# Parcels-code/Parcels

Hardware: AMD Instinct MI355X
Metric: RK4 particle-steps/sec (higher is better)
Workload: dtype f64

## Files before the change

### include/parcels_hip.h

```cpp
#ifndef PARCELS_HIP_H
#define PARCELS_HIP_H

#include <stdint.h>

#ifdef __cplusplus
extern "C" {
#endif

#define PK_ABI_VERSION 9
#define PK_MAX_GRIDS 4
#define PK_MAX_FIELDS 64
#define PK_MAX_KERNELS 8
#define PK_MAX_EXTRA 8
#define PK_NUM_STATE_CODES 80
#define PK_MAX_TWE 1024

typedef struct pk_ctx pk_ctx;

#define PK_F32 0
#define PK_F64 1
#define PK_I8 2
#define PK_U8 3
#define PK_I16 4
#define PK_U16 5
// ... 37 lines not shown
#define PK_KERNEL_USER0 40
#define PK_MAX_USER_KERNELS 8

int32_t pk_abi_version(void);
int32_t pk_init(int32_t device, pk_ctx** out);
int32_t pk_destroy(pk_ctx* ctx);
const char* pk_last_error(const pk_ctx* ctx);

int32_t pk_set_option(pk_ctx* ctx, const char* name, int32_t value);

int32_t pk_upload_stats(pk_ctx* ctx, double* out4);

int32_t pk_unpack_stats(pk_ctx* ctx, double* out4);

int32_t pk_host_stage_selftest(void);

typedef struct pk_device_info {
    char name[128];
    char arch[64];
    int32_t compute_units;
    int32_t wavefront_size;
    int32_t lds_bytes_per_block;
    int32_t clock_khz;
    int64_t total_mem;
    int64_t free_mem;
} pk_device_info;
int32_t pk_get_device_info(pk_ctx* ctx, pk_device_info* out);

typedef struct pk_grid_desc {
    int32_t kind;
// ... 316 lines not shown
```

### parcels_amd/_hip.py

```python

from __future__ import annotations

import ctypes as C
import os
import subprocess

_HERE = os.path.dirname(os.path.abspath(__file__))
LIB_PATH = os.environ.get("PARCELS_HIP_LIB", os.path.join(_HERE, "libparcels_hip.so"))

PK_ABI_VERSION = 9
PK_USER_RIDE, PK_USER_SAMPLES_UV, PK_USER_SAMPLES_UVW, PK_USER_UX, PK_USER_KEY_UX = 1, 2, 4, 8, 12
PK_USER_SIGMA, PK_USER_KEY_SIGMA = 16, 16
PK_F32, PK_F64 = 0, 1
PK_I8, PK_U8, PK_I16, PK_U16, PK_I32 = 2, 3, 4, 5, 6
PK_MAX_GRIDS, PK_MAX_FIELDS, PK_MAX_KERNELS, PK_NUM_STATE_CODES = 4, 64, 8, 80
PK_MAX_EXTRA = 8
PK_MAX_TWE = 1024
PK_KERNEL_SAMPLE_FIELD = 10
PK_KERNEL_ADVECTION_RK2_3D_CROCO = 11
PK_KERNEL_SAMPLE_SIGMA_CROCO = 12
PK_KERNEL_USER0 = 40
PK_EVAL_MASKED = 0x10000
PK_COMM_ID_BYTES = 128
PK_OP_MIN, PK_OP_MAX, PK_OP_SUM = 0, 1, 2
# ... 300 lines not shown
    "pk_interact_host_order",
    "pk_interact_sources",
    "pk_interact_prologue",
    "pk_interact_attract",
    "pk_interact_merge",
    "pk_interact_epilogue",
    "pk_particles_density",
    "pk_particles_cells",
    "pk_particles_connectivity",
    "pk_random_fill",
    "pk_measure_copy_bandwidth",
    "pk_set_option",
    "pk_upload_stats",
    "pk_unpack_stats",
    "pk_host_stage_selftest",
    "pk_particles_snapshot_filtered",
    "pk_comm_unique_id",
    "pk_comm_init",
    "pk_comm_destroy",
    "pk_comm_info",
    "pk_comm_allreduce_i64",
    "pk_comm_allgather_i64",
    "pk_gather_rows_to_root",
    "pk_allgather_output",
    "pk_gathered_fetch",
]

_lib = None


# ... 176 lines not shown
```

### parcels_amd/csrc/pk_api.hip

```cpp
#include "pk_api_ctx.h"

#include <rocprim/rocprim.hpp>

using namespace pkapi;

namespace pkapi {
std::string g_init_error;
}

namespace pk {

PK_DEV unsigned long long order_double(double v) {
    unsigned long long b = (unsigned long long)__double_as_longlong(v);
    return (b & 0x8000000000000000ull) ? ~b : (b | 0x8000000000000000ull);
}

__global__ void __launch_bounds__(64) clock_probe_kernel(unsigned long long* out, unsigned long long ticks) {
    if (threadIdx.x != 0) return;
    const unsigned long long r0 = __builtin_amdgcn_s_memrealtime();
    const unsigned long long c0 = __builtin_readcyclecounter();
    unsigned long long r = r0;
    while (r - r0 < ticks) {
        __builtin_amdgcn_s_sleep(8);
        r = __builtin_amdgcn_s_memrealtime();
// ... 341 lines not shown
        g_init_error = "device index out of range";
        return -2;
    }
    pk_ctx* ctx = new pk_ctx();
    ctx->device = device;
    if (const char* e = getenv("PK_SORT_HORIZONTAL")) ctx->sort_horizontal_major = atoi(e);
    if (const char* e = getenv("PK_NO_SPECIAL")) ctx->no_special = atoi(e);
    if (const char* e = getenv("PK_NO_CELL_CACHE")) ctx->no_cell_cache = atoi(e);
    if (const char* e = getenv("PK_NO_HASH_DIR")) ctx->no_hash_dir = atoi(e);
    if (const char* e = getenv("PK_NO_CELL_TABLE")) ctx->no_cell_table = atoi(e);
    if (const char* e = getenv("PK_NO_FAST")) ctx->no_fast = atoi(e);
    if (const char* e = getenv("PK_NO_FAST_CGRID")) ctx->no_fast_cgrid = atoi(e);
    if (const char* e = getenv("PK_NO_VELOCITY_PAIRS")) ctx->no_velocity_pairs = atoi(e);
    if (const char* e = getenv("PK_VELOCITY_PAIRS")) ctx->no_velocity_pairs = !atoi(e);
    ctx->no_block_cache = getenv("PK_NO_BLOCK_CACHE") != nullptr;
    *out = ctx;
    PK_HIP(ctx, hipSetDevice(device));
    PK_HIP(ctx, hipGetDeviceProperties(&ctx->prop, device));
    PK_HIP(ctx, hipStreamCreateWithFlags(&ctx->compute, hipStreamNonBlocking));
    PK_HIP(ctx, hipStreamCreateWithFlags(&ctx->copy, hipStreamNonBlocking));
    PK_HIP(ctx, hipEventCreate(&ctx->ev0));
    PK_HIP(ctx, hipEventCreate(&ctx->ev1));
    PK_HIP(ctx, hipEventCreate(&ctx->ev2));
    PK_HIP(ctx, hipEventCreate(&ctx->ev_p0));
    PK_HIP(ctx, hipEventCreate(&ctx->ev_p1));
    for (int k = 0; k < PK_STAGE_BUFFERS; k++) PK_HIP(ctx, hipEventCreateWithFlags(&ctx->stage_ev[k], hipEventDisableTiming));
    PK_HIP(ctx, hipMalloc((void**)&ctx->d_counters, sizeof(DCounters)));
    PK_HIP(ctx, hipMalloc((void**)&ctx->d_twe, sizeof(unsigned long long) * PK_MAX_TWE));
    PK_HIP(ctx, hipMalloc((void**)&ctx->d_twe_found, sizeof(unsigned long long) * TWE_FOUND_SLOTS));
    PK_HIP(ctx, hipMalloc((void**)&ctx->d_twe_hit, sizeof(unsigned int) * PK_MAX_TWE));
    PK_HIP(ctx, hipMalloc((void**)&ctx->d_summary, sizeof(unsigned long long) * (PK_NUM_STATE_CODES + 2)));
    PK_HIP(ctx, hipHostMalloc((void**)&ctx->h_counters, sizeof(DCounters), hipHostMallocDefault));
    PK_HIP(ctx, hipHostMalloc((void**)&ctx->h_summary, sizeof(unsigned long long) * (PK_NUM_STATE_CODES + 2), hipHostMallocDefault));
    PK_HIP(ctx, hipMalloc((void**)&ctx->d_clk, sizeof(unsigned long long) * 32));
    PK_HIP(ctx, hipMalloc((void**)&ctx->d_tstats, sizeof(unsigned long long) * 3));
    PK_HIP(ctx, hipHostMalloc((void**)&ctx->h_clk, sizeof(unsigned long long) * 32, hipHostMallocDefault));
    return 0;
}

int32_t pk_set_option(pk_ctx* ctx, const char* name, int32_t value) {
    if (!ctx || !name) return -2;
    const std::string n(name);
    if (n == "fast_path") ctx->no_fast = !value;
    else if (n == "fast_cgrid") ctx->no_fast_cgrid = !value;
    else if (n == "velocity_pairs") ctx->no_velocity_pairs = !value;
    else if (n == "clock_probe") ctx->clock_probe = value;
    else if (n == "special_programs") ctx->no_special = !value;
// ... 7 lines not shown
        ctx->block_cache = value;
    }
    else if (n == "miss_lanes") {
        if (value < -1 || value > 64) return ctx->fail("pk_set_option: miss_lanes is -1 (planned), 0 (never) or the most missing lanes of a wavefront, up to 64");
        ctx->miss_lanes = value;
    }
    else if (n == "fast_grid") {
        if (value < 0) return ctx->fail("pk_set_option: fast_grid is 0 (planned) or the largest number of workgroups of the persistent A-grid launch");
        ctx->fast_grid = value;
    }
    else if (n == "unpack_chunk_values") {
        if (value < 0) return ctx->fail("pk_set_option: unpack_chunk_values is 0 (what fits a staging chunk) or the most values per staged chunk of a packed level");
        ctx->unpack_chunk_values = value == 0 ? 0 : std::max(16, value / 16 * 16);
    }
    else if (n == "unpack_timing") ctx->unpack_timing = value != 0;
    else return ctx->fail("pk_set_option: unknown option '" + n + "'");
    return 0;
}

int32_t pk_upload_stats(pk_ctx* ctx, double* out4) {
    if (!ctx || !out4) return -2;
    out4[0] = ctx->stage_fill_s;
    out4[1] = ctx->stage_wait_s;
    out4[2] = ctx->stage_bytes_total;
    out4[3] = (double)pkhost::copy_threads();
    return 0;
}

static void free_snapshots(pk_ctx* ctx) {
    for (auto& sn : ctx->snap) {
        if (sn.in_flight && sn.done) (void)hipEventSynchronize(sn.done);
// ... 28 lines not shown
    for (hipEvent_t e : ctx->unpack_ev) (void)hipEventDestroy(e);
    for (hipEvent_t e : ctx->unpack_ev_free) (void)hipEventDestroy(e);
    if (ctx->tab_a.d) (void)hipFree(ctx->tab_a.d);
    if (ctx->tab_c.d) (void)hipFree(ctx->tab_c.d);
    if (ctx->d_ct2) (void)hipFree(ctx->d_ct2);
    if (ctx->d_vp) (void)hipFree(ctx->d_vp);
    if (ctx->d_sigma) (void)hipFree(ctx->d_sigma);
    if (ctx->d_counters) (void)hipFree(ctx->d_counters);
    if (ctx->d_twe) (void)hipFree(ctx->d_twe);
    if (ctx->d_twe_found) (void)hipFree(ctx->d_twe_found);
    if (ctx->d_twe_hit) (void)hipFree(ctx->d_twe_hit);
    if (ctx->d_desc) (void)hipFree(ctx->d_desc);
    if (ctx->h_desc) (void)hipHostFree(ctx->h_desc);
    if (ctx->d_summary) (void)hipFree(ctx->d_summary);
    if (ctx->h_counters) (void)hipHostFree(ctx->h_counters);
    if (ctx->h_summary) (void)hipHostFree(ctx->h_summary);
    (void)pk_comm_destroy(ctx);
    neighbors_free(ctx->nbr);
    interact_free(ctx->inter);
    if (ctx->sel.d_flag) (void)hipFree(ctx->sel.d_flag);
    if (ctx->sel.d_offs) (void)hipFree(ctx->sel.d_offs);
    if (ctx->sel.d_tmp) (void)hipFree(ctx->sel.d_tmp);
    if (ctx->d_clk) (void)hipFree(ctx->d_clk);
    if (ctx->d_tstats) (void)hipFree(ctx->d_tstats);
    if (ctx->h_clk) (void)hipHostFree(ctx->h_clk);
    for (int k = 0; k < PK_STAGE_BUFFERS; k++) {
        if (ctx->stage[k]) (void)hipHostFree(ctx->stage[k]);
        if (ctx->stage_ev[k]) (void)hipEventDestroy(ctx->stage_ev[k]);
    }
    if (ctx->ev0) (void)hipEventDestroy(ctx->ev0);
// ... 1304 lines not shown
    const CoordTable& T = ctx->tab_a;
    if (int32_t rc = coord_table(ctx, ctx->tab_a, U.d.grid, prm->fU, U.time.data(), f.has_time_interval ? f.nt : 0,
                                 {{g.d.depth, g.d.has_z ? g.d.nz : 0}, {g.d.lat, g.d.has_y ? g.d.ny : 0}, {g.d.lon, g.d.nx}}, 60 * 1024))
        return rc;
    if (!T.ok) return 0;
    const double inv_deg2m = 1.0 / g.d.deg2m;
    if (!(g.d.deg2m > 1e-100 && g.d.deg2m < 1e100) || !std::isfinite(inv_deg2m)) return 0;
    F.grid = U.d.grid;
    F.has_ti = f.has_time_interval;
    F.has_z = g.d.has_z; F.has_y = g.d.has_y; F.has_x = g.d.has_x;
    F.spherical = g.d.spherical;
    F.nt = f.nt;
    F.nslots = f.nslots;
    F.gnz = g.d.nz; F.gny = g.d.ny; F.gnx = g.d.nx;
    ravel_strides(g.d, F.ex, F.ey, F.ez);
    F.st_z = (uint32_t)f.st_z;
    F.st_y = (uint32_t)f.st_y;
    F.dyb = fy ? (uint32_t)(f.st_y * esz) : 0u;
    F.dzb = fz ? (uint32_t)(f.st_z * esz) : 0u;
    F.lds_time = T.off[0]; F.lds_depth = T.off[1]; F.lds_lat = T.off[2]; F.lds_lon = T.off[3];
    F.lds_n = T.off[4];
    F.lvl_b = (int64_t)lvl_b;
    F.U = (const char*)U.d.data; F.V = (const char*)V.d.data; F.W = W ? (const char*)W->d.data : nullptr;
    F.tab = T.d;
    F.tlen = f.tlen; F.t0 = f.tfirst; F.t1 = f.tlast;
    F.z0 = g.d.zfirst; F.z1 = g.d.zlast; F.y0 = g.d.yfirst; F.y1 = g.d.ylast; F.x0 = g.d.xfirst; F.x1 = g.d.xlast;
    F.deg2m = g.d.deg2m;
    F.inv_deg2m = inv_deg2m;
    F.ok = 1;
    return 0;
// ... 310 lines not shown
        p.lds = (size_t)a.fast.lds_n * 2 * sizeof(double);
        const bool lp_kernel = fast_prog == PROG_RK4 && !ride;
        const size_t lp_lds = (p.lds + (size_t)FAST_LP_BYTES + 2047) / 2048 * 2048;
        const bool lp_fits = 2 * lp_lds <= (size_t)160 * 1024;
        int mode = ctx->block_cache;
        if (ctx->no_block_cache && mode != 2) mode = 0;
        if (mode == 2 && !(lp_kernel && lp_fits))
            return ctx->fail(!lp_kernel ? "block_cache 2: only the library's 2-D A-grid kernel (AdvectionRK4 without user kernels) has the level-pair cache"
                                        : "block_cache 2: the coordinate tables leave no room for the level-pair cache at 16 waves per CU");
        if (mode < 0) mode = lp_kernel && lp_fits ? 2 : 1;
        if (mode == 2) {
            p.lp = FAST_LP_CACHE;
            a.fast.lds_blk = a.fast.lds_n;
            a.fast.miss_lanes = ctx->miss_lanes < 0 ? FAST_MISS_LANES_DEFAULT : ctx->miss_lanes;
            p.lds += (size_t)FAST_LP_BYTES;
        } else if (mode == 0 && lp_kernel && !ctx->no_block_cache) {
            p.lp = FAST_LP_REGS;
            a.fast.lds_blk = 0;
        } else {
            const bool blk = mode == 1 && fast_prog != PROG_RK4_3D && p.lds + (size_t)FAST_BLK_BYTES <= 64 * 1024;
            a.fast.lds_blk = blk ? a.fast.lds_n : 0;
            if (blk) p.lds += (size_t)FAST_BLK_BYTES;
        }
    } else {
        if (int32_t rc = fill_fastc(ctx, prm, a, fast_prog, prm->have_guess0 || us.assume_guessed, p.lds)) return rc;
        if (!a.fastc.ok) return 0;
        p.kernel = fast_prog == PROG_RK4_3D ? DEDICATED_C3 : DEDICATED_C2;
    }
    p.prog = fast_prog;
    p.ride = ride;
// ... 64 lines not shown
                stored++;
            }
            if (!stored) return ctx->fail("PK_KERNEL_SAMPLE_FIELD: every component is discarded");
        }
    }
    if (need_kh && (prm->fKh_zonal < 0 || prm->fKh_meridional < 0)) return ctx->fail("diffusion kernels need Kh_zonal/Kh_meridional");
    const HostField& U = ctx->fields[prm->fU];
    const int field_f32 = U.d.dtype == PK_F32;
    for (int f : {prm->fV, prm->fW})
        if (f >= 0 && ctx->fields[f].d.dtype != U.d.dtype) return ctx->fail("U, V, W must share one dtype");
    const int curv = ctx->grids[a.main_grid].d.kind == 1;
    const int64_t n = ctx->dev.n;
    if (prm->twe_n < 0 || prm->twe_n > PK_MAX_TWE || (prm->twe_n > 0 && !prm->twe_key)) return ctx->fail("params.twe_n / twe_key out of range");
    for (int k = 1; k < prm->twe_n; k++)
        if (!(prm->twe_key[k - 1] < prm->twe_key[k])) return ctx->fail("params.twe_key must be ascending");
    DCounters& counters0 = ctx->h_counters0;
    counters0 = DCounters{0ull, 0ull, 0ull, 0xFFFFFFFFu, 0u, ~0ull, 0u, 0u, {}, {}};
    PK_HIP(ctx, hipMemcpyAsync(ctx->d_counters, &counters0, sizeof(DCounters), hipMemcpyHostToDevice, ctx->compute));
    PK_HIP(ctx, hipMemsetAsync(ctx->d_twe_found, 0, sizeof(unsigned long long) * TWE_FOUND_SLOTS, ctx->compute));
    if (prm->twe_n > 0) PK_HIP(ctx, hipMemsetAsync(ctx->d_twe_hit, 0, sizeof(unsigned int) * prm->twe_n, ctx->compute));
    ctx->fl_twe_n = prm->twe_n;
    if (prm->twe_key != ctx->rerun_keys.data()) ctx->rerun_keys.assign(prm->twe_key, prm->twe_key + prm->twe_n);
    if (prm->twe_n > 0)
        PK_HIP(ctx, hipMemcpyAsync(ctx->d_twe, ctx->rerun_keys.data(), sizeof(int64_t) * prm->twe_n, hipMemcpyHostToDevice, ctx->compute));
    PK_HIP(ctx, hipMemsetAsync(ctx->d_summary, 0, sizeof(unsigned long long) * PK_NUM_STATE_CODES, ctx->compute));
    const unsigned long long init_mm[2] = {~0ull, 0ull};
    PK_HIP(ctx, hipMemcpyAsync(ctx->d_summary + PK_NUM_STATE_CODES, init_mm, sizeof(init_mm), hipMemcpyHostToDevice, ctx->compute));
    int launches = 0;
    bool sorted = false;
    if (n > 0) {
        const dim3 grid((unsigned)((n + 255) / 256));
        LaunchPlan p;
        rc = plan_launch(ctx, prm, UserShape{has_user, ctx->user_flags, ctx->user_nsample, ctx->user_sample_fid, false, false}, a, lds_bytes, use_lds, p);
        if (rc) return rc;
        if (has_user && p.prog == PROG_TYPED) return ctx->fail("user kernels run in the plain kernel-list interpreter only (float32 coordinate arrays are not supported)");
        if (p.kernel == DEDICATED_C2) ensure_velocity_pairs(ctx, prm, a.fastc);
        if (prm->sort_by_cell && !prm->body_only && p.prog != PROG_UX) {
            PK_HIP(ctx, hipEventRecord(ctx->ev2, ctx->compute));
            int horizontal = 1;
            for (int k = 0; k < prm->nk; k++)
                if (prm->kernels[k] == PK_KERNEL_ADVECTION_RK4_3D || prm->kernels[k] == PK_KERNEL_ADVECTION_RK2_3D) horizontal = 0;
            if (ctx->sort_horizontal_major >= 0) horizontal = ctx->sort_horizontal_major;
            rc = sort_particles(ctx, a.main_grid, horizontal);
            if (rc) return rc;
            a.p = ctx->dev;
            sorted = true;
        }
        rc = ensure_alt(ctx);
        if (rc) return rc;
        a.p = ctx->dev;
#define X(m, bit, elem, per_grid, optional) a.po.m = ctx->alt.m;
// ... 40 lines not shown
        }
        PK_HIP(ctx, hipGetLastError());
        PK_HIP(ctx, hipEventRecord(ctx->ev1, ctx->compute));
        if (ctx->clock_probe) {
            const unsigned long long us = ctx->clock_probe == 1 ? 1000ull : (unsigned long long)std::max(ctx->clock_probe, 20);
            hipLaunchKernelGGL(clock_probe_kernel, dim3(16), dim3(64), 0, ctx->probe, ctx->d_clk, us * 100ull);
            PK_HIP(ctx, hipMemcpyAsync(ctx->h_clk, ctx->d_clk, sizeof(unsigned long long) * 32, hipMemcpyDeviceToHost, ctx->probe));
        }
        ctx->fl_clock_probe = ctx->clock_probe != 0;
        launches = 1;
        ctx->fl_program = p.kernel == DEDICATED_NONE ? p.prog : (p.kernel <= DEDICATED_A3 ? PROGRAM_FAST_AGRID : PROGRAM_FAST_CGRID);
        swap_launch_outputs(ctx);
        ctx->rerun_valid = true;
        ctx->rerun_prm = *prm;
        ctx->rerun_prm.twe_key = nullptr;
        const unsigned sgrid = (unsigned)std::min<int64_t>((n + 255) / 256, 2048);
        hipLaunchKernelGGL(summarize_kernel, dim3(sgrid), dim3(256), 0, ctx->compute, ctx->dev.state, ctx->dev.t, n, ctx->d_summary);
        PK_HIP(ctx, hipGetLastError());
    }
    PK_HIP(ctx, hipMemcpyAsync(ctx->h_counters, ctx->d_counters, sizeof(DCounters), hipMemcpyDeviceToHost, ctx->compute));
    PK_HIP(ctx, hipMemcpyAsync(ctx->h_summary, ctx->d_summary, sizeof(unsigned long long) * (PK_NUM_STATE_CODES + 2), hipMemcpyDeviceToHost, ctx->compute));
    ctx->in_flight = true;
    ctx->fl_launches = launches;
    ctx->fl_sorted = sorted;
    ctx->fl_n = n;
    return 0;
}

int32_t pk_execute_end(pk_ctx* ctx, pk_exec_stats* stats) {
    if (!ctx) return -2;
    if (!ctx->in_flight) return ctx->fail("pk_execute_end: no launch in flight");
    PK_HIP(ctx, hipSetDevice(ctx->device));
    ctx->in_flight = false;
    PK_HIP(ctx, hipStreamSynchronize(ctx->compute));
    if (ctx->fl_clock_probe && ctx->probe) PK_HIP(ctx, hipStreamSynchronize(ctx->probe));
    {
// ... 5 lines not shown
            std::vector<unsigned long long> slots(TWE_FOUND_SLOTS);
            PK_HIP(ctx, hipMemcpy(slots.data(), ctx->d_twe_found, sizeof(unsigned long long) * TWE_FOUND_SLOTS, hipMemcpyDeviceToHost));
            for (unsigned long long k : slots)
                if (k) ctx->twe_found_host.push_back((int64_t)k);
            std::sort(ctx->twe_found_host.begin(), ctx->twe_found_host.end());
        }
        if (ctx->fl_launches && ctx->fl_twe_n > 0) {
            std::vector<unsigned int> hit((size_t)ctx->fl_twe_n);
            PK_HIP(ctx, hipMemcpy(hit.data(), ctx->d_twe_hit, sizeof(unsigned int) * ctx->fl_twe_n, hipMemcpyDeviceToHost));
            for (int k = 0; k < ctx->fl_twe_n; k++) ctx->twe_hit_host[k] = hit[k] ? 1 : 0;
        }
    }
    if (stats) {
        memset(stats, 0, sizeof(*stats));
        const DCounters& hc = *ctx->h_counters;
        const unsigned long long* hs = ctx->h_summary;
        stats->steps = (int64_t)hc.steps;
        stats->attempts = (int64_t)hc.attempts;
        stats->paused = (int64_t)hc.paused;
        for (int k = 0; k < PK_NUM_STATE_CODES; k++) stats->state_counts[k] = (int64_t)hs[k];
        auto unorder = [](unsigned long long o) {
            unsigned long long b = (o & 0x8000000000000000ull) ? (o & 0x7fffffffffffffffull) : ~o;
            double v;
            memcpy(&v, &b, 8);
            return v;
        };
        const bool any_live = ctx->fl_n > 0 && hs[PK_EVALUATE] > 0;
        stats->t_min_live = any_live ? unorder(hs[PK_NUM_STATE_CODES]) : NAN;
        stats->t_max_live = any_live ? unorder(hs[PK_NUM_STATE_CODES + 1]) : NAN;
        float ms = 0.f;
        if (ctx->fl_launches) PK_HIP(ctx, hipEventElapsedTime(&ms, ctx->ev0, ctx->ev1));
// ... 138 lines not shown
```

### parcels_amd/csrc/pk_api_ctx.h

```cpp
#pragma once
#include <hip/hip_runtime.h>

#include <algorithm>
#include <array>
#include <chrono>
#include <cmath>
#include <cstdio>
#include <cstdlib>
#include <cstring>
#include <string>
#include <thread>
#include <vector>

#include "pk_hashbuild.h"
#include "pk_neighbors.h"
#include "pk_interact.h"
#include "pk_density.h"
#include "pk_connectivity.h"
#include "pk_host_stage.h"
#include "pk_kernels.h"
#include "pk_ux.h"
#include "pk_sigma.h"

using namespace pk;
// ... 117 lines not shown
    int fl_launches = 0;
    int fl_program = 0;
    bool rerun_valid = false;
    pk_exec_params rerun_prm{};
    void (*user_launch)(const void*, int32_t, int32_t, int32_t, uint64_t, void*) = nullptr;
    int32_t user_flags = 0;
    int32_t user_nsample = 0;
    int32_t user_sample_fid[4] = {0, 0, 0, 0};
    char* d_chk = nullptr;
    size_t chk_bytes = 0;
    bool chk_valid = false, chk_has_perm = false;
    int64_t chk_n = 0;
    bool fl_sorted = false;
    int64_t fl_n = 0;
    DCounters* h_counters = nullptr;
    DCounters h_counters0;
    unsigned long long* d_twe = nullptr;
    unsigned long long* d_twe_found = nullptr;
    unsigned int* d_twe_hit = nullptr;
    std::vector<int64_t> twe_found_host;
    std::vector<uint8_t> twe_hit_host;
    bool twe_overflow_host = false;
    int fl_twe_n = 0;
    std::vector<int64_t> rerun_keys;
    unsigned long long* h_summary = nullptr;
    unsigned long long* d_tstats = nullptr;
    unsigned long long* d_clk = nullptr;
    unsigned long long* h_clk = nullptr;
    double* d_sigma = nullptr;
    SigmaA sigma{};
    bool has_sigma = false;
    int sort_horizontal_major = -1;
    int no_special = 0;
    bool eval_points_f32 = false;
    int no_cell_cache = 0;
    int no_hash_dir = 0;
    int no_cell_table = 0;
    int no_fast = 0;
    int no_fast_cgrid = 0;
    bool no_block_cache = false;
    int block_cache = -1;
    int miss_lanes = -1;
    int fast_grid = 0;
    struct Snapshot {
        void* dev[PK_NCOLS] = {};
        void* host[PK_NCOLS] = {};
        int64_t capacity = 0;
        int64_t n = 0;
        uint32_t mask = 0;
        int ngrids = 0;
        size_t ss = 0;
        size_t extra_elem[PK_MAX_EXTRA] = {};
        hipEvent_t ready = nullptr, done = nullptr;
        bool in_flight = false;
    } snap[2];
    CoordTable tab_a, tab_c;
// ... 83 lines not shown
```

### parcels_amd/csrc/pk_device.h

```cpp
#pragma once
#include <hip/hip_runtime.h>
#include <stdint.h>

#include "../../include/parcels_hip.h"

namespace pk {

struct DGrid {
    int32_t kind, spherical;
    int32_t has_x, has_y, has_z;
    int32_t nx, ny, nz;
    int32_t xdim, ydim, zdim;
    int32_t off_x, off_y, off_z;
    int32_t lon_f32, lat_f32, depth_f32;
    int32_t h_bitwidth;
    double deg2m;
    const double* lon;
    const double* lat;
    const double* depth;
    const double* node_tab;
    const double* cell_tab;
    const uint32_t* h_keys;
    const int64_t* h_starts;
    const int64_t* h_counts;
// ... 40 lines not shown
    void *z, *y, *x, *dz, *dy, *dx;
    double* dt;
    double* next_dt;
    int32_t* state;
    int32_t* ei;
    int32_t* iter;
};

struct DCounters {
    unsigned long long steps, attempts, paused;
    unsigned int err_iter, pad;
    unsigned long long twe_key;
    unsigned int twe_overflow, pad2;
    unsigned int pad3[20];
    unsigned int cursor[8 * 32];
};
constexpr int PK_CURSOR_STRIDE = 32;
static_assert(offsetof(DCounters, cursor) == 128, "the cursors start on a line of their own");

struct FastA {
    int32_t ok, grid;
    int32_t has_ti, has_z, has_y, has_x, spherical;
    int32_t nt, nslots;
    int32_t gnz, gny, gnx;
    uint32_t ex, ey, ez;
    uint32_t st_z, st_y;
    uint32_t dyb, dzb;
    int32_t lds_time, lds_depth, lds_lat, lds_lon, lds_n;
    int32_t lds_blk;
    int64_t lvl_b;
    const char *U, *V, *W;
    const double* tab;
    double tlen, t0, t1, z0, z1, y0, y1, x0, x1;
    double deg2m, inv_deg2m;
    int32_t ns;
    int32_t miss_lanes;
    int32_t sfid[4];
    const char* S[4];
};

struct FastC {
    int32_t ok, grid;
    int32_t has_ti, has_z, walk_ok, near_edges;
    int32_t nt, nslots;
    int32_t gnz, gny, gnx;
    uint32_t ex, ey, ez;
    int32_t lds_time, lds_depth, lds_n;
    int32_t lds_rec, lds_fv;
    int32_t st_z, st_y;
    int32_t cb;
    int64_t lvl_b;
    int64_t dU0, dU1, dV0, dV1;
    union { int64_t dW0; int64_t vp_slot_b; };
// ... 25 lines not shown
    double win_lo, win_hi;
    DCounters* counters;
    const unsigned long long* twe_listed;
    unsigned long long* twe_found;
    unsigned int* twe_hit;
    int32_t lds_time, lds_depth, lds_lat, lds_lon, lds_total;
    int32_t lds_cc_nodes, lds_cc_keys, lds_cc_fvals;
    int32_t main_grid, main_field;
    DPOut po;
    union {
        FastA fast;
        FastC fastc;
        SigmaA sigma;
    };
};

#define PK_DEV __device__ __forceinline__
PK_DEV const DGrid& kgrid(const KArgs& a, int g) { return *(const DGrid*)(a.grids + g); }
PK_DEV const DField& kfield(const KArgs& a, int f) { return *(const DField*)(a.fields + f); }
PK_DEV unsigned long long twe_sample_key(unsigned it, int klo) { return ((unsigned long long)it << 32) | (unsigned long long)(unsigned)klo; }
PK_DEV bool twe_listed(const KArgs& a, unsigned it, int klo) {
    const int n = a.prm.twe_n;
    if (__builtin_expect(n == 0, 1)) return false;
    const unsigned long long key = twe_sample_key(it, klo);
    const unsigned long long* lst = a.twe_listed;
    int lo = 0, hi = n;
    while (lo < hi) {
        const int mid = (lo + hi) >> 1;
        if (lst[mid] < key) lo = mid + 1; else hi = mid;
    }
// ... 1468 lines not shown
```

### parcels_amd/csrc/pk_fast_agrid.h

```cpp
#pragma once
#include "pk_device.h"

namespace pk {

typedef double pk_tab2 __attribute__((ext_vector_type(2)));

struct FastTabs {
    const pk_tab2* time;
    const pk_tab2* depth;
    const pk_tab2* lat;
    const pk_tab2* lon;
    pk_tab2* blk;
    uint32_t fl;
    double tlen;
    int32_t gny, gnx;
    double deg2m, inv_deg2m;
};
PK_DEV void copy_scalars(FastTabs& T, const FastA& F) {
    T.tlen = F.tlen;
    T.gny = F.gny;
    T.gnx = F.gnx;
}
enum : uint32_t {
    FA_TI = 1u, FA_Z = 2u, FA_Y = 4u, FA_X = 8u, FA_SPH = 16u, FA_RING = 32u, FA_BLK = 64u,
// ... 378 lines not shown
    int state;
    int32_t ei;
    int ht, hz, hy, hx;
    int zi;
    uint32_t zez;
    double mt, mtau, mz, mzeta;
    int32_t bei;
    int32_t bkey;
    double ya, yb, yr, xa, xb, xr;
    LpField fu, fv;
    double ta, tb, tr;
};
constexpr int32_t FAST_NO_BLOCK = -0x7fffffff - 1;
constexpr int FAST_Z_UNSEARCHED = -3;
constexpr int FAST_Z_UNSEARCHED_PACKED = -0x7fffffff - 1;
PK_DEV void fctx_depth_moved(FCtx& c, bool held) {
    c.zi = held ? FAST_Z_UNSEARCHED_PACKED : FAST_Z_UNSEARCHED;
    c.ya = __builtin_inf();
}
PK_DEV void fctx_init(FCtx& c, int state, int32_t ei, bool cache, bool held) {
    c.state = state;
    c.ei = ei;
    c.ht = c.hz = c.hy = c.hx = 0;
    c.zi = held ? FAST_Z_UNSEARCHED_PACKED : cache ? FAST_Z_UNSEARCHED : 0;
    c.ya = c.xa = c.ta = __builtin_inf();
    c.yb = c.xb = c.yr = c.xr = c.tb = c.tr = 0.0;
    c.zez = 0u;
    c.mt = c.mz = __builtin_nan("");
    c.mtau = c.mzeta = 0.0;
    c.bei = FAST_NO_BLOCK;
// ... 161 lines not shown
            tau = c.mtau;
        }
        ti = c.ht;
    }
    int zi = 0, yi = 0, xi = 0;
    double zeta = 0.0, eta = 0.0, xsi = 0.0;
    auto depth_zeta = [&]() -> double {
        if ((fl & (FA_Z | FA_NZ2)) != (FA_Z | FA_NZ2)) return 0.0;
        const int q = c.zi >> 1;
        const int h = q >= 0 ? q : (q == LEFT_OUT_OF_BOUNDS ? 0 : F.gnz - 2);
        const pk_tab2 e = T.depth[h];
        return fast_bary(z, e.x, T.depth[h + 1].x, e.y);
    };
    if (fl & FA_Z) {
        if constexpr (HELD) {
            if (c.zi == FAST_Z_UNSEARCHED_PACKED) {
                int hz = 0, idx;
                double bz;
                fast_search<true>(T.depth, F.gnz, F.z0, F.z1, z, hz, idx, bz, (fl & FA_NZ2) != 0);
                c.zi = idx * 2 + (!(bz <= 0) ? 1 : 0);
                c.bei = FAST_NO_BLOCK;
            }
            zi = c.zi >> 1;
        } else {
            if (CACHE ? c.zi == FAST_Z_UNSEARCHED : !(z == c.mz)) {
                fast_depth_search(T, F, c, fl, z, !CACHE);
            }
            zi = c.zi;
            zeta = c.mzeta;
        }
    }
    if constexpr (CACHE) {
// ... 167 lines not shown
```

### parcels_amd/csrc/pk_kernels.h

```cpp
#pragma once
#include "pk_device.h"
#include "pk_fast_agrid.h"
#include "pk_fast_cgrid.h"

namespace pk {

static_assert(sizeof(KArgs) <= 4096, "kernel arguments must fit the 4 KiB kernarg segment");

enum Program { PROG_RK4 = 0, PROG_RK4_3D = 1, PROG_GENERIC = 2, PROG_RK45 = 3, PROG_M1 = 4, PROG_TYPED = 5 };

struct PState {
    double t, z, y, x, dz, dy, dx, dt, next_dt;
    int64_t id;
};

PK_DEV double ldp(const void* col, int64_t i, bool pf) { return pf ? (double)((const float*)col)[i] : ((const double*)col)[i]; }
PK_DEV void stp(void* col, int64_t i, double v, bool pf) {
    if (pf) ((float*)col)[i] = (float)v; else ((double*)col)[i] = v;
}
PK_DEV double padd(bool pf, double a, double b) { return pf ? (double)((float)a + (float)b) : a + b; }
PK_DEV double psub(bool pf, double a, double b) { return pf ? (double)((float)a - (float)b) : a - b; }
PK_DEV double pstore(bool pf, double v) { return pf ? (double)(float)v : v; }

enum { RQ_UV = 0, RQ_UVW = 1, RQ_SCALAR = 2, RQ_VEC = 3 };
// ... 331 lines not shown
    return v;
}

PK_DEV unsigned long long uniform_u64(unsigned long long v) {
    const unsigned lo = (unsigned)__builtin_amdgcn_readfirstlane((int)(unsigned)v), hi = (unsigned)__builtin_amdgcn_readfirstlane((int)(unsigned)(v >> 32));
    return ((unsigned long long)hi << 32) | lo;
}

PK_DEV unsigned xcd_swizzle(unsigned bid, unsigned nb) {
    const unsigned xcd = bid & 7u, j = bid >> 3;
    const unsigned per = nb >> 3, rem = nb & 7u;
    return xcd * per + (xcd < rem ? xcd : rem) + j;
}

constexpr int FAST_CHUNK = 64;
PK_DEV bool fast_claim(DCounters* cnt, unsigned nchunks, unsigned& tried, unsigned& chunk) {
    const unsigned per = nchunks >> 3, rem = nchunks & 7u;
    while (tried < 8u) {
        const unsigned s = (blockIdx.x + tried) & 7u;
        unsigned k = 0u;
        if ((threadIdx.x & 63) == 0) k = atomicAdd(&cnt->cursor[s * PK_CURSOR_STRIDE], 1u);
        k = (unsigned)__builtin_amdgcn_readfirstlane((int)k);
        if (k < per + (s < rem ? 1u : 0u)) {
            chunk = s * per + (s < rem ? s : rem) + k;
            return true;
        }
        tried++;
    }
    return false;
}
// ... 278 lines not shown
}
#endif

#ifndef PK_MIN_WAVES_FAST
#define PK_MIN_WAVES_FAST 4
#endif
template <class FT, int PFM, bool D3, int LP = FAST_LP_OFF>
__global__ void __launch_bounds__(fast_wg(LP), PK_MIN_WAVES_FAST) advect_fast_kernel(const KArgs a) {
    extern __shared__ __attribute__((aligned(16))) double smem[];
    constexpr int WG = fast_wg(LP);
    FastTabs ft;
    {
        pk_tab2* s_tab = reinterpret_cast<pk_tab2*>(smem);
        const pk_tab2* g_tab = reinterpret_cast<const pk_tab2*>(a.fast.tab);
        for (int k = threadIdx.x; k < a.fast.lds_n; k += WG) s_tab[k] = g_tab[k];
        __syncthreads();
        ft.time = s_tab + a.fast.lds_time;
        ft.depth = s_tab + a.fast.lds_depth;
        ft.lat = s_tab + a.fast.lds_lat;
        ft.lon = s_tab + a.fast.lds_lon;
        ft.blk = s_tab + a.fast.lds_blk + threadIdx.x;
        copy_scalars(ft, a.fast);
        ft.fl = fast_flags(a.fast) | ((a.win_lo > -INFINITY || a.win_hi < INFINITY) ? FA_WIN : 0u) | (a.prm.dt0 > 0 ? FA_FWD : 0u) |
                (a.prm.max_iters > 0 ? FA_MAXIT : 0u);
        if constexpr (fast_held(LP, PFM == 1)) ft.fl |= (uint32_t)a.fast.miss_lanes << FA_MISS_LANES_SHIFT;
    }
    constexpr bool PERS = LP == FAST_LP_CACHE;
    [[maybe_unused]] unsigned chunk = 0u, tried = 0u;
    [[maybe_unused]] const unsigned nchunks = PERS ? (unsigned)((a.p.n + FAST_CHUNK - 1) / FAST_CHUNK) : 0u;
    auto row = [&]() {
        if constexpr (PERS) {
            unsigned tid = threadIdx.x;
            asm volatile("" : "+v"(tid));
            return (int64_t)chunk * FAST_CHUNK + (tid & 63u);
        } else return (int64_t)xcd_swizzle(blockIdx.x, gridDim.x) * WG + threadIdx.x;
    };
    [[maybe_unused]] unsigned long long all_steps = 0ull, all_attempts = 0ull, all_paused = 0ull;
    do {
        if constexpr (PERS) {
            if (!fast_claim(a.counters, nchunks, tried, chunk)) break;
        }
        unsigned steps = 0, attempts = 0, paused = 0;
        if (row() < a.p.n) {
            int64_t i = row();
            const DParticles& P = a.p;
            const DPOut& O = a.po;
            const pk_exec_params& prm = a.prm;
            constexpr bool pf = PFM == 1;
            FCtx c;
            c.state = prm.reset_state ? PK_EVALUATE : P.state[i];
            if (c.state == PK_EVALUATE) {
                unsigned it = prm.reset_state ? 0u : (unsigned)P.iter[i];
                fctx_init(c, PK_EVALUATE, P.ei[i * P.ngrids + a.fast.grid], LP == FAST_LP_CACHE, fast_held(LP, pf));
                double pt = P.t[i];
                double pz = ldp(P.z, i, pf), py = ldp(P.y, i, pf), px = ldp(P.x, i, pf);
                double pdz = ldp(P.dz, i, pf), pdy = ldp(P.dy, i, pf), pdx = ldp(P.dx, i, pf);
                double pdt = P.dt[i];
                const double endtime = prm.endtime;
                while (c.state == PK_EVALUATE) {
                    uint32_t fl = ft.fl;
                    asm volatile("" : "+s"(fl));
                    if constexpr (fast_held(LP, pf)) {
                        ft.deg2m = a.fast.deg2m;
                        ft.inv_deg2m = a.fast.inv_deg2m;
                        asm volatile("" : "+s"(ft.deg2m), "+s"(ft.inv_deg2m));
                    }
                    const bool fwd = (fl & FA_FWD) != 0;
                    const double tte = fwd ? endtime - pt : -(endtime - pt);
// ... 73 lines not shown
                            break;
                        }
                        px = padd(pf, px, pdx);
                        py = padd(pf, py, pdy);
                        if constexpr (LP == FAST_LP_CACHE) {
                            if (__builtin_expect(!(pdz == 0), 0)) fctx_depth_moved(c, fast_held(LP, pf));
                        }
                        pz = padd(pf, pz, pdz);
                        pt += pdt;
                        pdx = pdy = pdz = 0.0;
                        steps++;
                    }
                    pdt = prm.dt0;
                    if (c.state == PK_EVALUATE && pt == endtime) c.state = PK_ENDOFLOOP;
                }
                i = row();
                asm volatile("" : "+v"(i));
                O.t[i] = pt;
                stp(O.z, i, pz, pf);
                stp(O.y, i, py, pf);
                stp(O.x, i, px, pf);
                stp(O.dz, i, pdz, pf);
                stp(O.dy, i, pdy, pf);
                stp(O.dx, i, pdx, pf);
                O.dt[i] = pdt;
                if (P.next_dt && O.next_dt != P.next_dt) O.next_dt[i] = P.next_dt[i];
                O.state[i] = c.state;
                for (int g = 0; g < P.ngrids; g++) O.ei[i * P.ngrids + g] = g == a.fast.grid ? c.ei : P.ei[i * P.ngrids + g];
                O.iter[i] = (int32_t)it;
                note_error_iteration(a, c.state, it);
            }
        }
        unsigned long long wsteps = wave_sum((unsigned long long)steps), wattempts = wave_sum((unsigned long long)attempts),
                           wpaused = wave_sum((unsigned long long)paused);
        if constexpr (PERS) {
            all_steps += uniform_u64(wsteps);
            all_attempts += uniform_u64(wattempts);
            all_paused += uniform_u64(wpaused);
            continue;
        }
        if ((threadIdx.x & 63) == 0) {
            if (wsteps) atomicAdd(&a.counters->steps, wsteps);
            if (wattempts) atomicAdd(&a.counters->attempts, wattempts);
            if (wpaused) atomicAdd(&a.counters->paused, wpaused);
        }
    } while (PERS);
    if constexpr (PERS) {
        if ((threadIdx.x & 63) == 0) {
            if (all_steps) atomicAdd(&a.counters->steps, all_steps);
            if (all_attempts) atomicAdd(&a.counters->attempts, all_attempts);
            if (all_paused) atomicAdd(&a.counters->paused, all_paused);
        }
    }
}


#ifndef PK_MIN_WAVES_CGRID
#define PK_MIN_WAVES_CGRID 3
#endif
#ifndef PK_MIN_WAVES_CGRID_RK45
#define PK_MIN_WAVES_CGRID_RK45 3
#endif
#ifndef PK_MIN_WAVES_CGRID_M1
#define PK_MIN_WAVES_CGRID_M1 3
#endif
#ifndef PK_CG_CACHE
// ... 578 lines not shown
```

Baseline: 52.30 billion.

## Fuse end-of-step state summary into persistent A-grid kernel via LDS histogram

The persistent dedicated A-grid kernel now accumulates the per-state particle histogram and the min/max time of evaluating particles in an LDS table as each chunk finishes. It flushes that table to a summary area appended to the counters block, which removes the separate summarize kernel launch, its memsets, and its extra pass over the state and time arrays. The counter reset now copies from pinned host memory. Warm search hints and a uniform-sum shortcut are added behind compile flags that are off by default. The cost is extra LDS per block, LDS and global atomics, and a wider counters struct to copy back.

```diff
diff --git a/include/parcels_hip.h b/include/parcels_hip.h
--- a/include/parcels_hip.h
+++ b/include/parcels_hip.h
@@ -75,6 +75,8 @@
 int32_t pk_unpack_stats(pk_ctx* ctx, double* out4);
 
 int32_t pk_host_stage_selftest(void);
+
+int32_t pk_fast_unravel_hints(uint32_t ey, uint32_t ez, int32_t gnz, int32_t gny, int32_t gnx, const int32_t* ei, int64_t n, int32_t* out3);
 
 typedef struct pk_device_info {
     char name[128];
diff --git a/parcels_amd/_hip.py b/parcels_amd/_hip.py
--- a/parcels_amd/_hip.py
+++ b/parcels_amd/_hip.py
@@ -338,6 +338,7 @@
     "pk_upload_stats",
     "pk_unpack_stats",
     "pk_host_stage_selftest",
+    "pk_fast_unravel_hints",
     "pk_particles_snapshot_filtered",
     "pk_comm_unique_id",
     "pk_comm_init",
diff --git a/parcels_amd/csrc/pk_api.hip b/parcels_amd/csrc/pk_api.hip
--- a/parcels_amd/csrc/pk_api.hip
+++ b/parcels_amd/csrc/pk_api.hip
@@ -379,6 +379,7 @@
     if (const char* e = getenv("PK_NO_VELOCITY_PAIRS")) ctx->no_velocity_pairs = atoi(e);
     if (const char* e = getenv("PK_VELOCITY_PAIRS")) ctx->no_velocity_pairs = !atoi(e);
     ctx->no_block_cache = getenv("PK_NO_BLOCK_CACHE") != nullptr;
+    if (const char* e = getenv("PK_FUSED_SUMMARY")) ctx->fused_summary = atoi(e) != 0;
     *out = ctx;
     PK_HIP(ctx, hipSetDevice(device));
     PK_HIP(ctx, hipGetDeviceProperties(&ctx->prop, device));
@@ -396,6 +397,9 @@
     PK_HIP(ctx, hipMalloc((void**)&ctx->d_twe_hit, sizeof(unsigned int) * PK_MAX_TWE));
     PK_HIP(ctx, hipMalloc((void**)&ctx->d_summary, sizeof(unsigned long long) * (PK_NUM_STATE_CODES + 2)));
     PK_HIP(ctx, hipHostMalloc((void**)&ctx->h_counters, sizeof(DCounters), hipHostMallocDefault));
+    PK_HIP(ctx, hipHostMalloc((void**)&ctx->h_counters0, sizeof(DCounters), hipHostMallocDefault));
+    *ctx->h_counters0 = DCounters{0ull, 0ull, 0ull, 0xFFFFFFFFu, 0u, ~0ull, 0u, 0u, {}, {}, {}};
+    ctx->h_counters0->summary[PK_NUM_STATE_CODES] = ~0ull;
     PK_HIP(ctx, hipHostMalloc((void**)&ctx->h_summary, sizeof(unsigned long long) * (PK_NUM_STATE_CODES + 2), hipHostMallocDefault));
     PK_HIP(ctx, hipMalloc((void**)&ctx->d_clk, sizeof(unsigned long long) * 32));
     PK_HIP(ctx, hipMalloc((void**)&ctx->d_tstats, sizeof(unsigned long long) * 3));
@@ -433,7 +437,19 @@
         ctx->unpack_chunk_values = value == 0 ? 0 : std::max(16, value / 16 * 16);
     }
     else if (n == "unpack_timing") ctx->unpack_timing = value != 0;
+    else if (n == "fused_summary") ctx->fused_summary = value != 0;
     else return ctx->fail("pk_set_option: unknown option '" + n + "'");
+    return 0;
+}
+
+int32_t pk_fast_unravel_hints(uint32_t ey, uint32_t ez, int32_t gnz, int32_t gny, int32_t gnx, const int32_t* ei, int64_t n, int32_t* out3) {
+    if (n < 0 || (n > 0 && (!ei || !out3))) return -2;
+    const uint32_t my = fast_magic(ey), mz = fast_magic(ez);
+    for (int64_t k = 0; k < n; k++) {
+        int zi, yi, xi;
+        fast_unravel((uint32_t)ei[k], ey, ez, my, mz, gnz, gny, gnx, zi, yi, xi);
+        out3[3 * k] = zi; out3[3 * k + 1] = yi; out3[3 * k + 2] = xi;
+    }
     return 0;
 }
 
@@ -492,6 +508,7 @@
     if (ctx->h_desc) (void)hipHostFree(ctx->h_desc);
     if (ctx->d_summary) (void)hipFree(ctx->d_summary);
     if (ctx->h_counters) (void)hipHostFree(ctx->h_counters);
+    if (ctx->h_counters0) (void)hipHostFree(ctx->h_counters0);
     if (ctx->h_summary) (void)hipHostFree(ctx->h_summary);
     (void)pk_comm_destroy(ctx);
     neighbors_free(ctx->nbr);
@@ -1826,6 +1843,9 @@
     F.nslots = f.nslots;
     F.gnz = g.d.nz; F.gny = g.d.ny; F.gnx = g.d.nx;
     ravel_strides(g.d, F.ex, F.ey, F.ez);
+    F.ey_magic = fast_magic(F.ey);
+    F.ez_magic = fast_magic(F.ez);
+    F.fused_summary = 0;
     F.st_z = (uint32_t)f.st_z;
     F.st_y = (uint32_t)f.st_y;
     F.dyb = fy ? (uint32_t)(f.st_y * esz) : 0u;
@@ -2166,6 +2186,11 @@
             a.fast.lds_blk = a.fast.lds_n;
             a.fast.miss_lanes = ctx->miss_lanes < 0 ? FAST_MISS_LANES_DEFAULT : ctx->miss_lanes;
             p.lds += (size_t)FAST_LP_BYTES;
+            const size_t with_sum = (p.lds + (size_t)FAST_SUM_BYTES + 2047) / 2048 * 2048;
+            if (PK_FAST_FUSED_SUMMARY != 0 && ctx->fused_summary && 2 * with_sum <= (size_t)160 * 1024) {
+                a.fast.fused_summary = 1;
+                p.lds += (size_t)FAST_SUM_BYTES;
+            }
         } else if (mode == 0 && lp_kernel && !ctx->no_block_cache) {
             p.lp = FAST_LP_REGS;
             a.fast.lds_blk = 0;
@@ -2260,27 +2285,30 @@
     if (prm->twe_n < 0 || prm->twe_n > PK_MAX_TWE || (prm->twe_n > 0 && !prm->twe_key)) return ctx->fail("params.twe_n / twe_key out of range");
     for (int k = 1; k < prm->twe_n; k++)
         if (!(prm->twe_key[k - 1] < prm->twe_key[k])) return ctx->fail("params.twe_key must be ascending");
-    DCounters& counters0 = ctx->h_counters0;
-    counters0 = DCounters{0ull, 0ull, 0ull, 0xFFFFFFFFu, 0u, ~0ull, 0u, 0u, {}, {}};
-    PK_HIP(ctx, hipMemcpyAsync(ctx->d_counters, &counters0, sizeof(DCounters), hipMemcpyHostToDevice, ctx->compute));
+    PK_HIP(ctx, hipMemcpyAsync(ctx->d_counters, ctx->h_counters0, sizeof(DCounters), hipMemcpyHostToDevice, ctx->compute));
     PK_HIP(ctx, hipMemsetAsync(ctx->d_twe_found, 0, sizeof(unsigned long long) * TWE_FOUND_SLOTS, ctx->compute));
     if (prm->twe_n > 0) PK_HIP(ctx, hipMemsetAsync(ctx->d_twe_hit, 0, sizeof(unsigned int) * prm->twe_n, ctx->compute));
     ctx->fl_twe_n = prm->twe_n;
     if (prm->twe_key != ctx->rerun_keys.data()) ctx->rerun_keys.assign(prm->twe_key, prm->twe_key + prm->twe_n);
     if (prm->twe_n > 0)
         PK_HIP(ctx, hipMemcpyAsync(ctx->d_twe, ctx->rerun_keys.data(), sizeof(int64_t) * prm->twe_n, hipMemcpyHostToDevice, ctx->compute));
-    PK_HIP(ctx, hipMemsetAsync(ctx->d_summary, 0, sizeof(unsigned long long) * PK_NUM_STATE_CODES, ctx->compute));
-    const unsigned long long init_mm[2] = {~0ull, 0ull};
-    PK_HIP(ctx, hipMemcpyAsync(ctx->d_summary + PK_NUM_STATE_CODES, init_mm, sizeof(init_mm), hipMemcpyHostToDevice, ctx->compute));
     int launches = 0;
-    bool sorted = false;
+    bool sorted = false, fused = false;
+    LaunchPlan p;
     if (n > 0) {
-        const dim3 grid((unsigned)((n + 255) / 256));
-        LaunchPlan p;
         rc = plan_launch(ctx, prm, UserShape{has_user, ctx->user_flags, ctx->user_nsample, ctx->user_sample_fid, false, false}, a, lds_bytes, use_lds, p);
         if (rc) return rc;
         if (has_user && p.prog == PROG_TYPED) return ctx->fail("user kernels run in the plain kernel-list interpreter only (float32 coordinate arrays are not supported)");
         if (p.kernel == DEDICATED_C2) ensure_velocity_pairs(ctx, prm, a.fastc);
+        fused = p.kernel == DEDICATED_A2 && !p.ride && p.lp == FAST_LP_CACHE && a.fast.fused_summary != 0;
+    }
+    if (!fused) {
+        PK_HIP(ctx, hipMemsetAsync(ctx->d_summary, 0, sizeof(unsigned long long) * PK_NUM_STATE_CODES, ctx->compute));
+        const unsigned long long init_mm[2] = {~0ull, 0ull};
+        PK_HIP(ctx, hipMemcpyAsync(ctx->d_summary + PK_NUM_STATE_CODES, init_mm, sizeof(init_mm), hipMemcpyHostToDevice, ctx->compute));
+    }
+    if (n > 0) {
+        const dim3 grid((unsigned)((n + 255) / 256));
         if (prm->sort_by_cell && !prm->body_only && p.prog != PROG_UX) {
             PK_HIP(ctx, hipEventRecord(ctx->ev2, ctx->compute));
             int horizontal = 1;
@@ -2351,12 +2379,17 @@
         ctx->rerun_valid = true;
         ctx->rerun_prm = *prm;
         ctx->rerun_prm.twe_key = nullptr;
-        const unsigned sgrid = (unsigned)std::min<int64_t>((n + 255) / 256, 2048);
-        hipLaunchKernelGGL(summarize_kernel, dim3(sgrid), dim3(256), 0, ctx->compute, ctx->dev.state, ctx->dev.t, n, ctx->d_summary);
-        PK_HIP(ctx, hipGetLastError());
+    }
+    if (!fused) {
+        if (n > 0) {
+            const unsigned sgrid = (unsigned)std::min<int64_t>((n + 255) / 256, 2048);
+            hipLaunchKernelGGL(summarize_kernel, dim3(sgrid), dim3(256), 0, ctx->compute, ctx->dev.state, ctx->dev.t, n, ctx->d_summary);
+            PK_HIP(ctx, hipGetLastError());
+        }
+        PK_HIP(ctx, hipMemcpyAsync(ctx->h_summary, ctx->d_summary, sizeof(unsigned long long) * (PK_NUM_STATE_CODES + 2), hipMemcpyDeviceToHost, ctx->compute));
     }
     PK_HIP(ctx, hipMemcpyAsync(ctx->h_counters, ctx->d_counters, sizeof(DCounters), hipMemcpyDeviceToHost, ctx->compute));
-    PK_HIP(ctx, hipMemcpyAsync(ctx->h_summary, ctx->d_summary, sizeof(unsigned long long) * (PK_NUM_STATE_CODES + 2), hipMemcpyDeviceToHost, ctx->compute));
+    ctx->fl_fused_summary = fused;
     ctx->in_flight = true;
     ctx->fl_launches = launches;
     ctx->fl_sorted = sorted;
@@ -2392,7 +2425,7 @@
     if (stats) {
         memset(stats, 0, sizeof(*stats));
         const DCounters& hc = *ctx->h_counters;
-        const unsigned long long* hs = ctx->h_summary;
+        const unsigned long long* hs = ctx->fl_fused_summary ? hc.summary : ctx->h_summary;
         stats->steps = (int64_t)hc.steps;
         stats->attempts = (int64_t)hc.attempts;
         stats->paused = (int64_t)hc.paused;
diff --git a/parcels_amd/csrc/pk_api_ctx.h b/parcels_amd/csrc/pk_api_ctx.h
--- a/parcels_amd/csrc/pk_api_ctx.h
+++ b/parcels_amd/csrc/pk_api_ctx.h
@@ -155,7 +155,7 @@
     bool fl_sorted = false;
     int64_t fl_n = 0;
     DCounters* h_counters = nullptr;
-    DCounters h_counters0;
+    DCounters* h_counters0 = nullptr;
     unsigned long long* d_twe = nullptr;
     unsigned long long* d_twe_found = nullptr;
     unsigned int* d_twe_hit = nullptr;
@@ -181,6 +181,8 @@
     int no_fast_cgrid = 0;
     bool no_block_cache = false;
     int block_cache = -1;
+    int fused_summary = 1;
+    bool fl_fused_summary = false;
     int miss_lanes = -1;
     int fast_grid = 0;
     struct Snapshot {
diff --git a/parcels_amd/csrc/pk_device.h b/parcels_amd/csrc/pk_device.h
--- a/parcels_amd/csrc/pk_device.h
+++ b/parcels_amd/csrc/pk_device.h
@@ -78,9 +78,11 @@
     unsigned int twe_overflow, pad2;
     unsigned int pad3[20];
     unsigned int cursor[8 * 32];
+    unsigned long long summary[PK_NUM_STATE_CODES + 2];
 };
 constexpr int PK_CURSOR_STRIDE = 32;
 static_assert(offsetof(DCounters, cursor) == 128, "the cursors start on a line of their own");
+static_assert(offsetof(DCounters, summary) == 128 + 8 * 32 * 4, "the summary words lie behind the cursors");
 
 struct FastA {
     int32_t ok, grid;
@@ -101,6 +103,8 @@
     int32_t miss_lanes;
     int32_t sfid[4];
     const char* S[4];
+    uint32_t ey_magic, ez_magic;
+    int32_t fused_summary;
 };
 
 struct FastC {
@@ -156,6 +160,7 @@
         SigmaA sigma;
     };
 };
+static_assert(sizeof(FastA) <= sizeof(FastC), "the kernel arguments keep their size: FastA grows inside the union only");
 
 #define PK_DEV __device__ __forceinline__
 PK_DEV const DGrid& kgrid(const KArgs& a, int g) { return *(const DGrid*)(a.grids + g); }
diff --git a/parcels_amd/csrc/pk_fast_agrid.h b/parcels_amd/csrc/pk_fast_agrid.h
--- a/parcels_amd/csrc/pk_fast_agrid.h
+++ b/parcels_amd/csrc/pk_fast_agrid.h
@@ -416,6 +416,11 @@
 constexpr int32_t FAST_NO_BLOCK = -0x7fffffff - 1;
 constexpr int FAST_Z_UNSEARCHED = -3;
 constexpr int FAST_Z_UNSEARCHED_PACKED = -0x7fffffff - 1;
+#ifndef PK_FAST_WARM_HINTS
+#define PK_FAST_WARM_HINTS 0
+#endif
+constexpr int FAST_Z_HINT_END = FAST_Z_UNSEARCHED_PACKED + 0x10000;
+PK_DEV int fctx_depth_hint_packed(int h) { return FAST_Z_UNSEARCHED_PACKED + h; }
 PK_DEV void fctx_depth_moved(FCtx& c, bool held) {
     c.zi = held ? FAST_Z_UNSEARCHED_PACKED : FAST_Z_UNSEARCHED;
     c.ya = __builtin_inf();
@@ -607,8 +612,8 @@
     };
     if (fl & FA_Z) {
         if constexpr (HELD) {
-            if (c.zi == FAST_Z_UNSEARCHED_PACKED) {
-                int hz = 0, idx;
+            if (PK_FAST_WARM_HINTS != 0 ? c.zi < FAST_Z_HINT_END : c.zi == FAST_Z_UNSEARCHED_PACKED) {
+                int hz = PK_FAST_WARM_HINTS != 0 ? c.zi - FAST_Z_UNSEARCHED_PACKED : 0, idx;
                 double bz;
                 fast_search<true>(T.depth, F.gnz, F.z0, F.z1, z, hz, idx, bz, (fl & FA_NZ2) != 0);
                 c.zi = idx * 2 + (!(bz <= 0) ? 1 : 0);
diff --git a/parcels_amd/csrc/pk_kernels.h b/parcels_amd/csrc/pk_kernels.h
--- a/parcels_amd/csrc/pk_kernels.h
+++ b/parcels_amd/csrc/pk_kernels.h
@@ -369,6 +369,75 @@
 }
 
 constexpr int FAST_CHUNK = 64;
+#ifndef PK_FAST_WARM_HINTS
+#define PK_FAST_WARM_HINTS 0
+#endif
+#ifndef PK_FAST_UNIFORM_SUMS
+#define PK_FAST_UNIFORM_SUMS 0
+#endif
+#ifndef PK_FAST_FUSED_SUMMARY
+#define PK_FAST_FUSED_SUMMARY 1
+#endif
+inline uint32_t fast_magic(uint32_t d) { return d == 0u ? 0u : (d == 1u ? 0xFFFFFFFFu : (uint32_t)((1ull << 32) / d)); }
+__host__ __device__ __forceinline__ uint32_t fast_divmod_magic(uint32_t n, uint32_t d, uint32_t m, uint32_t& rem) {
+#ifdef __HIP_DEVICE_COMPILE__
+    uint32_t q = __umulhi(n, m);
+#else
+    uint32_t q = (uint32_t)(((unsigned long long)n * m) >> 32);
+#endif
+    uint32_t r = n - q * d;
+    if (m != 0u && r >= d) { q++; r -= d; }
+    rem = r;
+    return q;
+}
+__host__ __device__ __forceinline__ void fast_unravel(uint32_t ei, uint32_t ey, uint32_t ez, uint32_t ey_magic, uint32_t ez_magic, int gnz, int gny, int gnx,
+                                                      int& zi, int& yi, int& xi) {
+    uint32_t r, x;
+    const uint32_t z = fast_divmod_magic(ei, ez, ez_magic, r);
+    const uint32_t y = fast_divmod_magic(r, ey, ey_magic, x);
+    auto cell = [](uint32_t v, int n) { return (int)(v < (uint32_t)(n > 2 ? n - 2 : 0) ? v : (uint32_t)(n > 2 ? n - 2 : 0)); };
+    zi = cell(z, gnz);
+    yi = cell(y, gny);
+    xi = cell(x, gnx);
+}
+constexpr int FAST_SUM_WORDS = PK_NUM_STATE_CODES + 4;
+constexpr int FAST_SUM_BYTES = FAST_SUM_WORDS * 4;
+static_assert(FAST_SUM_BYTES % 16 == 0 && PK_NUM_STATE_CODES % 2 == 0, "whole table entries; the 64-bit words are aligned");
+PK_DEV unsigned* fast_summary_words(double* smem, const FastA& F) {
+    return reinterpret_cast<unsigned*>(reinterpret_cast<pk_tab2*>(smem) + F.lds_blk) + FAST_LP_BYTES / 4;
+}
+PK_DEV unsigned long long fast_order_double(double v) {
+    const unsigned long long b = (unsigned long long)__double_as_longlong(v);
+    return (b & 0x8000000000000000ull) ? ~b : (b | 0x8000000000000000ull);
+}
+PK_DEV void fast_summary_chunk(unsigned* words, int state, double t) {
+    const int s0 = __builtin_amdgcn_readfirstlane(state);
+    if (__builtin_amdgcn_ballot_w64(state != s0 && state != -1) == 0ull) {
+        const unsigned cnt = (unsigned)__builtin_popcountll(__builtin_amdgcn_ballot_w64(state == s0));
+        if (s0 >= 0 && s0 < PK_NUM_STATE_CODES && (threadIdx.x & 63) == 0) atomicAdd(&words[s0], cnt);
+    } else if (state >= 0 && state < PK_NUM_STATE_CODES) {
+        atomicAdd(&words[state], 1u);
+    }
+    if (state == PK_EVALUATE) {
+        unsigned long long* mm = reinterpret_cast<unsigned long long*>(words + PK_NUM_STATE_CODES);
+        const unsigned long long o = fast_order_double(t);
+        atomicMin(&mm[0], o);
+        atomicMax(&mm[1], o);
+    }
+}
+PK_DEV void fast_summary_flush(unsigned* words, DCounters* cnt) {
+    __syncthreads();
+    const int k = threadIdx.x;
+    if (k < PK_NUM_STATE_CODES) {
+        if (words[k]) atomicAdd(&cnt->summary[k], (unsigned long long)words[k]);
+    } else if (k == PK_NUM_STATE_CODES) {
+        const unsigned long long* mm = reinterpret_cast<const unsigned long long*>(words + PK_NUM_STATE_CODES);
+        if (mm[0] != ~0ull || mm[1] != 0ull) {
+            atomicMin(&cnt->summary[PK_NUM_STATE_CODES], mm[0]);
+            atomicMax(&cnt->summary[PK_NUM_STATE_CODES + 1], mm[1]);
+        }
+    }
+}
 PK_DEV bool fast_claim(DCounters* cnt, unsigned nchunks, unsigned& tried, unsigned& chunk) {
     const unsigned per = nchunks >> 3, rem = nchunks & 7u;
     while (tried < 8u) {
@@ -677,6 +746,12 @@
         pk_tab2* s_tab = reinterpret_cast<pk_tab2*>(smem);
         const pk_tab2* g_tab = reinterpret_cast<const pk_tab2*>(a.fast.tab);
         for (int k = threadIdx.x; k < a.fast.lds_n; k += WG) s_tab[k] = g_tab[k];
+        if constexpr (LP == FAST_LP_CACHE && PK_FAST_FUSED_SUMMARY != 0) {
+            if (a.fast.fused_summary) {
+                unsigned* hist = fast_summary_words(smem, a.fast);
+                for (int k = threadIdx.x; k < FAST_SUM_WORDS; k += WG) hist[k] = (k == PK_NUM_STATE_CODES || k == PK_NUM_STATE_CODES + 1) ? ~0u : 0u;
+            }
+        }
         __syncthreads();
         ft.time = s_tab + a.fast.lds_time;
         ft.depth = s_tab + a.fast.lds_depth;
@@ -699,11 +774,14 @@
         } else return (int64_t)xcd_swizzle(blockIdx.x, gridDim.x) * WG + threadIdx.x;
     };
     [[maybe_unused]] unsigned long long all_steps = 0ull, all_attempts = 0ull, all_paused = 0ull;
+    [[maybe_unused]] int warm_ht = 0;
     do {
         if constexpr (PERS) {
             if (!fast_claim(a.counters, nchunks, tried, chunk)) break;
         }
         unsigned steps = 0, attempts = 0, paused = 0;
+        [[maybe_unused]] int end_state = -1;
+        [[maybe_unused]] double end_t = 0.0;
         if (row() < a.p.n) {
             int64_t i = row();
             const DParticles& P = a.p;
@@ -712,9 +790,17 @@
             constexpr bool pf = PFM == 1;
             FCtx c;
             c.state = prm.reset_state ? PK_EVALUATE : P.state[i];
+            if constexpr (PERS && PK_FAST_FUSED_SUMMARY != 0) end_state = c.state;
             if (c.state == PK_EVALUATE) {
                 unsigned it = prm.reset_state ? 0u : (unsigned)P.iter[i];
                 fctx_init(c, PK_EVALUATE, P.ei[i * P.ngrids + a.fast.grid], LP == FAST_LP_CACHE, fast_held(LP, pf));
+                if constexpr (PERS && PK_FAST_WARM_HINTS != 0) {
+                    int wz;
+                    fast_unravel((uint32_t)c.ei, a.fast.ey, a.fast.ez, a.fast.ey_magic, a.fast.ez_magic, a.fast.gnz, a.fast.gny, a.fast.gnx, wz, c.hy, c.hx);
+                    c.ht = warm_ht;
+                    if constexpr (fast_held(LP, pf)) c.zi = fctx_depth_hint_packed(wz);
+                    else c.hz = wz;
+                }
                 double pt = P.t[i];
                 double pz = ldp(P.z, i, pf), py = ldp(P.y, i, pf), px = ldp(P.x, i, pf);
                 double pdz = ldp(P.dz, i, pf), pdy = ldp(P.dy, i, pf), pdx = ldp(P.dx, i, pf);
@@ -818,6 +904,8 @@
                     pdt = prm.dt0;
                     if (c.state == PK_EVALUATE && pt == endtime) c.state = PK_ENDOFLOOP;
                 }
+                if constexpr (PERS && PK_FAST_WARM_HINTS != 0) warm_ht = __builtin_amdgcn_readfirstlane(c.ht);
+                if constexpr (PERS && PK_FAST_FUSED_SUMMARY != 0) { end_state = c.state; end_t = pt; }
                 i = row();
                 asm volatile("" : "+v"(i));
                 O.t[i] = pt;
@@ -835,6 +923,19 @@
                 note_error_iteration(a, c.state, it);
             }
         }
+        if constexpr (PERS && PK_FAST_FUSED_SUMMARY != 0) {
+            if (a.fast.fused_summary) fast_summary_chunk(fast_summary_words(smem, a.fast), end_state, end_t);
+        }
+        if constexpr (PERS && PK_FAST_UNIFORM_SUMS != 0) {
+            const unsigned s0 = (unsigned)__builtin_amdgcn_readfirstlane((int)steps), a0 = (unsigned)__builtin_amdgcn_readfirstlane((int)attempts);
+            const unsigned long long like0 = __builtin_amdgcn_ballot_w64(steps == s0 && attempts == a0 && paused == 0u);
+            if ((like0 | __builtin_amdgcn_ballot_w64((steps | attempts | paused) == 0u)) == ~0ull) {
+                const unsigned long long lanes = (unsigned long long)__builtin_popcountll(like0);
+                all_steps += s0 * lanes;
+                all_attempts += a0 * lanes;
+                continue;
+            }
+        }
         unsigned long long wsteps = wave_sum((unsigned long long)steps), wattempts = wave_sum((unsigned long long)attempts),
                            wpaused = wave_sum((unsigned long long)paused);
         if constexpr (PERS) {
@@ -854,6 +955,9 @@
             if (all_steps) atomicAdd(&a.counters->steps, all_steps);
             if (all_attempts) atomicAdd(&a.counters->attempts, all_attempts);
             if (all_paused) atomicAdd(&a.counters->paused, all_paused);
+        }
+        if constexpr (PK_FAST_FUSED_SUMMARY != 0) {
+            if (a.fast.fused_summary) fast_summary_flush(fast_summary_words(smem, a.fast), a.counters);
         }
     }
 }
```

After: 52.86 billion, median of 6. +1.1%, better.
